# huzaifakhan04/truely-real-time-ai-generated-video-detection-framework-for-social-platforms

Measured on AMD Instinct MI355X. Metric: frames/sec (detect+embed+drift) 720p, higher is better.
Workload: dtype f32; 1 GPU; BASELINE configs[1]: synthetic 720p 1-face frames, batch=256 per GPU, fp32, MTCNN detect + 80x80 crop + InceptionResnetV1 embed + cosine drift score; frames_per_gpu=256, height=720, width=1280, weights=seeded synthetic (no checkpoints offline), prelu_slopes=unit, min_face_size=20, pyramid_levels=11, valid_faces=256, score=6, emb_crc32=3015932725, mode=sharded, ingest=resident, parallelism=single GPU, batches_in_flight=1, driver=single, embed_group=8

## Files before the change

__graft_entry__.py:

```python
import os
import subprocess
import sys

ROOT = os.path.dirname(os.path.abspath(__file__))
PKG = os.path.join(ROOT, "truely-real-time-ai-generated-video-detection-framework-for-social-platforms_amd")
if ROOT not in sys.path:
    sys.path.insert(0, ROOT)


def build() -> None:
    subprocess.check_call(["make", "-C", os.path.join(PKG, "csrc"), "-j4", "-s"])
    subprocess.check_call(["make", "-C", os.path.join(ROOT, "oracle"), "-s"])
    import truely_amd
    from truely_amd import _lib
    lib = _lib.load()
    missing = [n for n in _lib.EXPORTS if not hasattr(lib, n)]
    if missing:
        raise RuntimeError(f"libtruely_hip.so lacks {missing}")


def smoke() -> None:
    import numpy as np
    import torch
    import truely_amd
    from truely_amd.engine import Engine
    from oracle.oracle import Oracle
    assert torch.cuda.is_available(), "smoke() needs cuda:0"
    torch.cuda.set_device(0)
    blob = truely_amd.weights.synthetic_blob(0)
    eng = Engine(blob, device=0)
    frames = truely_amd.synthetic.synthetic_frames(4, 180, 320, seed=3)
    out = eng.detect_embed(frames)
    d = eng.drift_score(out["emb"], out["valid"], 16, 30)
    ref = Oracle(blob).detect_embed(frames)
    assert np.array_equal(out["valid"].cpu().numpy(), ref["valid"]), "valid mask differs from the oracle"
    assert np.array_equal(out["rect"].cpu().numpy(), ref["rect"]), "crop rectangles differ from the oracle"
    err = float(np.abs(out["emb"].cpu().numpy() - ref["emb"]).max())
    assert err <= 1e-4, f"embedding error {err}"
    assert "libtruely_hip.so" in open("/proc/self/maps").read()
    print(f"smoke ok: {int(ref['valid'].sum())}/4 faces, max |emb - oracle| = {err:.3g}, score = {d['score']}")


if __name__ == "__main__":
    build()
# ... 3 lines not shown
```

include/truely_hip.h:

```cpp
#ifndef TRUELY_HIP_H
#define TRUELY_HIP_H
#include <stddef.h>
#include <stdint.h>

#ifdef __cplusplus
extern "C" {
#endif

#define TRL_ABI_VERSION 7

typedef enum {
    TRL_OK = 0,
    TRL_ERR_INVALID = -1,
    TRL_ERR_HIP = -2,
    TRL_ERR_WEIGHTS = -3,
    TRL_ERR_CAPACITY = -4,
    TRL_ERR_STATE = -5
} trl_status;

typedef struct trl_ctx trl_ctx;

typedef struct {
    int    device;
    int    min_face_size;
// ... 41 lines not shown
                      void* stream);

int  trl_detect_crop(trl_ctx* ctx, const uint8_t* d_frames, int n, int H, int W,
                     float* d_box, float* d_prob, int32_t* d_rect, uint8_t* d_valid, float* d_faces, void* stream);
int  trl_facenet_embed_masked(trl_ctx* ctx, const float* d_faces, const uint8_t* d_valid, int n, int h, int w, float* d_emb, void* stream);

int  trl_detect_embed_begin(trl_ctx* ctx, const uint8_t* d_frames, int n, int H, int W,
                            float* d_box, float* d_prob, int32_t* d_rect, uint8_t* d_valid, float* d_emb, void* stream);
int  trl_detect_crop_begin(trl_ctx* ctx, const uint8_t* d_frames, int n, int H, int W,
                           float* d_box, float* d_prob, int32_t* d_rect, uint8_t* d_valid, float* d_faces, void* stream);
int  trl_detect_embed_end(trl_ctx* ctx);

int  trl_drift_score(trl_ctx* ctx, const float* d_emb, const uint8_t* d_valid, int n,
                     long long frame_count, int fps, float* d_sims, uint8_t* d_flags,
                     int32_t* d_result, void* stream);

#define TRL_DRIFT_STATE_BYTES 2064
int  trl_drift_update(trl_ctx* ctx, void* d_state, const float* d_emb, const uint8_t* d_valid, int n,
                      long long frame_count, int fps, float* d_sims, uint8_t* d_flags, int32_t* d_result, void* stream);

int  trl_ingest_nv12(trl_ctx* ctx, const uint8_t* d_nv12, int n_in, int H, int W, int step,
                     uint8_t* d_bgr, int* n_out, void* stream);
int  trl_ingest_i420(trl_ctx* ctx, const uint8_t* d_i420, int n_in, int H, int W, int step,
                     uint8_t* d_bgr, int* n_out, void* stream);

int  trl_debug_stage_boxes(trl_ctx* ctx, int stage, int frame, float* h_boxes, int max_rows, int* n_out);
int  trl_debug_level_counts(trl_ctx* ctx, int frame, int32_t* h_cand, int32_t* h_keep, int* n_levels);
int  trl_debug_level_cands(trl_ctx* ctx, int frame, int level, void* h_rows, int max_rows, int* n_out);
int  trl_debug_level_keep(trl_ctx* ctx, int frame, int level, int32_t* h_idx, int max_rows, int* n_out);
int  trl_debug_nms_tiers(trl_ctx* ctx, int small_tier, int full_tier);
int  trl_debug_list_stats(trl_ctx* ctx, long long* h_out8);
int  trl_debug_option(trl_ctx* ctx, const char* key, int value);
int  trl_debug_pnet_screen_bound(trl_ctx* ctx, float* A, float* B, int* on);
int  trl_debug_batch_capacity(trl_ctx* ctx, float t2_per_frame, float t3_per_frame, int* last_attempts);
int  trl_debug_pyramid_level(trl_ctx* ctx, const uint8_t* d_frame, int H, int W, int level, float* d_out, int* h, int* w, void* stream);
int  trl_debug_pyramid_batch(trl_ctx* ctx, const uint8_t* d_frames, int n, int H, int W, float* d_out, long long* pyr_stride,
                             int32_t* h_levels, int max_levels, int* n_levels, void* stream);
#define TRL_PYR_PLAN_COLS 6
enum { TRL_PYR_FINE = 1, TRL_PYR_S4 = 2, TRL_PYR_S8 = 3, TRL_PYR_SW4 = 4, TRL_PYR_SW8 = 5,
       TRL_PYR_L0_3 = 6, TRL_PYR_L0_4 = 7, TRL_PYR_L0_5 = 8, TRL_PYR_L1 = 9, TRL_PYR_L2 = 10 };
int  trl_debug_pyramid_plan(trl_ctx* ctx, int32_t* h_rows, int max_levels, int* n_levels);
enum { TRL_FNK_FN_CONV = 1, TRL_FNK_FN_SPLIT4 = 2, TRL_FNK_CONV_TAP = 3, TRL_FNK_IGEMM_VEC = 4, TRL_FNK_IGEMM_SCALAR = 5,
       TRL_FNK_SPLITK4 = 6, TRL_FNK_SPLITK4_TAP = 7, TRL_FNK_TAP48 = 8, TRL_FNK_BF16 = 9 };
typedef struct {
    int32_t conv, family, bm, bn, bk, pad, nz, m, cout, k, precision, has_res;
    char layer[48];
} trl_fn_plan_row;
int  trl_debug_facenet_plan(trl_ctx* ctx, trl_fn_plan_row* h_rows, int max_rows, int* n_rows);
int  trl_debug_facenet_capture(trl_ctx* ctx, int conv_index);
int  trl_debug_facenet_capture_read(trl_ctx* ctx, int view, void* h_dst, size_t max_bytes, int32_t* dims5);
int  trl_debug_poison(trl_ctx* ctx, int byte);
int  trl_debug_pnet_level(trl_ctx* ctx, const uint8_t* d_frame, int H, int W, int level,
                          float* d_prob, float* d_reg, int* oh, int* ow, void* stream);
int  trl_debug_rnet(trl_ctx* ctx, const float* d_crops, int n, float* d_out, void* stream);
int  trl_debug_onet(trl_ctx* ctx, const float* d_crops, int n, float* d_out, void* stream);
int  trl_debug_front_net(trl_ctx* ctx, const uint8_t* d_frame, int H, int W, const float* h_boxes, int nb, int net,
                         float* d_out, void* stream);
int  trl_debug_stage_net(trl_ctx* ctx, const uint8_t* d_frames, int nf, int H, int W, const float* h_recs, int nb, int net,
                         int capacity, float* d_out, void* stream);
int  trl_debug_front(trl_ctx* ctx, const uint8_t* d_frames, int nf, int H, int W, const int32_t* h_win, int nb, int net,
                     int capacity, float* d_pool, void* stream);
int  trl_debug_lists(trl_ctx* ctx, int kind, int n, int H, int W, const int32_t* h_caps, int n_levels, const int32_t* h_counts,
                     const void* h_rows, const float* h_logits, float* h_pts, float* d_boxes, float* d_probs, float* d_points,
                     int32_t* d_counts, float* d_box0, float* d_prob0, int32_t* d_rect, uint8_t* d_valid, void* stream);
int  trl_debug_mtcnn_plan(trl_ctx* ctx, trl_fn_plan_row* h_rows, int max_rows, int* n_rows);
int  trl_debug_crop_resize(trl_ctx* ctx, const uint8_t* d_frames, int n, int H, int W,
// ... 105 lines not shown
```

truely-real-time-ai-generated-video-detection-framework-for-social-platforms_amd/_lib.py:

```python
from __future__ import annotations

import ctypes as C
import os

_HERE = os.path.dirname(os.path.abspath(__file__))
LIB_PATH = os.path.join(_HERE, "libtruely_hip.so")


class TrlConfig(C.Structure):
    _fields_ = [("device", C.c_int), ("min_face_size", C.c_int), ("thr0", C.c_float), ("thr1", C.c_float),
                ("thr2", C.c_float), ("factor", C.c_double), ("cap_level", C.c_int), ("cap_frame", C.c_int),
                ("max_faces", C.c_int), ("pnet_mode", C.c_int), ("embed_mode", C.c_int), ("embed_precision", C.c_int)]


class TrlJpegdInfo(C.Structure):
    _fields_ = [(n, C.c_int32) for n in ("width", "height", "h_samp", "v_samp", "restart_interval", "scan_offset", "supported", "reason")]


class TrlJpegOptions(C.Structure):
    _fields_ = [(n, C.c_int) for n in ("quality", "subsampling", "restart_rows", "restart_blocks", "optimize")]


class TrlRzHit(C.Structure):
    _fields_ = [("arena", C.c_int32), ("block", C.c_int32), ("site", C.c_char * 24)] + \
# ... 41 lines not shown
    "trl_debug_level_keep": (C.c_int, [_vp, _i, _i, _vp, _i, C.POINTER(_i)]),
    "trl_debug_batch_capacity": (C.c_int, [_vp, _f, _f, C.POINTER(_i)]),
    "trl_debug_nms_tiers": (C.c_int, [_vp, _i, _i]),
    "trl_debug_option": (C.c_int, [_vp, C.c_char_p, _i]),
    "trl_debug_list_stats": (C.c_int, [_vp, C.POINTER(C.c_longlong)]),
    "trl_debug_poison": (C.c_int, [_vp, _i]),
    "trl_debug_pyramid_level": (C.c_int, [_vp, _vp, _i, _i, _i, _vp, C.POINTER(_i), C.POINTER(_i), _vp]),
    "trl_debug_pyramid_batch": (C.c_int, [_vp, _vp, _i, _i, _i, _vp, C.POINTER(C.c_longlong), _vp, _i, C.POINTER(_i), _vp]),
    "trl_debug_pyramid_plan": (C.c_int, [_vp, _vp, _i, C.POINTER(_i)]),
    "trl_debug_facenet_plan": (C.c_int, [_vp, _vp, _i, C.POINTER(_i)]),
    "trl_debug_facenet_capture": (C.c_int, [_vp, _i]),
    "trl_debug_facenet_capture_read": (C.c_int, [_vp, _i, _vp, C.c_size_t, _vp]),
    "trl_debug_pnet_level": (C.c_int, [_vp, _vp, _i, _i, _i, _vp, _vp, C.POINTER(_i), C.POINTER(_i), _vp]),
    "trl_debug_rnet": (C.c_int, [_vp, _vp, _i, _vp, _vp]),
    "trl_debug_onet": (C.c_int, [_vp, _vp, _i, _vp, _vp]),
    "trl_debug_front_net": (C.c_int, [_vp, _vp, _i, _i, _vp, _i, _i, _vp, _vp]),
    "trl_debug_stage_net": (C.c_int, [_vp, _vp, _i, _i, _i, _vp, _i, _i, _i, _vp, _vp]),
    "trl_debug_front": (C.c_int, [_vp, _vp, _i, _i, _i, _vp, _i, _i, _i, _vp, _vp]),
    "trl_debug_mtcnn_plan": (C.c_int, [_vp, _vp, _i, C.POINTER(_i)]),
    "trl_debug_lists": (C.c_int, [_vp, _i, _i, _i, _i, _vp, _i, _vp, _vp, _vp, _vp, _vp, _vp, _vp, _vp, _vp, _vp, _vp, _vp, _vp]),
    "trl_debug_crop_resize": (C.c_int, [_vp, _vp, _i, _i, _i, _vp, _vp, _vp, _vp]),
    "trl_debug_crop_aligned": (C.c_int, [_vp, _vp, _i, _i, _i, _vp, _vp, _i, _i, _vp, _vp]),
    "trl_debug_crop_area": (C.c_int, [_vp, _vp, _i, _i, _i, _vp, _vp, _i, _i, _vp, _vp]),
    "trl_debug_timings": (C.c_int, [_vp, C.POINTER(_f)]),
    "trl_debug_workspace": (C.c_int, [_vp, _i, _i, _i, _i, C.POINTER(C.c_longlong)]),
    "trl_debug_redzone": (C.c_int, [_vp, C.c_longlong, _i]),
    "trl_debug_redzone_report": (C.c_int, [_vp, _i, C.POINTER(C.c_longlong), C.POINTER(TrlRzHit), _i]),
    "trl_debug_redzone_poke": (C.c_int, [_vp, _i, _i, C.c_longlong, _i]),
    "trl_debug_stage_totals": (C.c_int, [_vp, C.POINTER(C.c_int32)]),
    "trl_debug_pnet_run": (C.c_int, [_vp, _i]),
    "trl_debug_pnet_kernel_ms": (C.c_int, [_vp, C.POINTER(C.c_float)]),
    "trl_debug_pnet_span": (C.c_int, [_vp, C.c_int, C.POINTER(C.c_double), C.POINTER(C.c_int32)]),
    "trl_debug_pnet_screen_bound": (C.c_int, [_vp, C.POINTER(_f), C.POINTER(_f), C.POINTER(_i)]),
    "trl_jpeg_create": (C.c_int, [_i, _i, _i, _i, _i, C.POINTER(_vp)]),
    "trl_jpeg_destroy": (C.c_int, [_vp]),
    "trl_jpeg_encode": (C.c_int, [_vp, _vp, _i, C.c_longlong, _vp, C.c_longlong, _vp, _vp]),
    "trl_jpeg_header": (C.c_int, [_i, _i, _i, _vp, C.c_size_t, C.POINTER(_i)]),
    "trl_jpeg_create_ex": (C.c_int, [_i, _i, _i, C.POINTER(TrlJpegOptions), _i, C.POINTER(_vp)]),
    "trl_jpeg_header_ex": (C.c_int, [_i, _i, C.POINTER(TrlJpegOptions), _vp, C.c_size_t, C.POINTER(_i)]),
    "trl_jpeg_optimal_table": (C.c_int, [_vp, _vp, _vp, C.POINTER(_i), C.POINTER(_i)]),
    "trl_jpegd_parse": (C.c_int, [_vp, C.c_size_t, _vp]),
    "trl_jpegd_create": (C.c_int, [_i, _i, _i, _i, C.c_longlong, C.POINTER(_vp)]),
    "trl_jpegd_destroy": (C.c_int, [_vp]),
    "trl_jpegd_debug_poison": (C.c_int, [_vp, _i]),
    "trl_jpegd_decode": (C.c_int, [_vp, _vp, _vp, _vp, _vp, _i, _vp, C.c_longlong, _vp, _vp]),
    "trl_draw_workspace": (C.c_size_t, [_i, _i]),
    "trl_draw": (C.c_int, [_vp, _i, C.c_longlong, _i, _i, _vp, _i, _vp, _i, _vp, C.c_size_t, _vp]),
    "trl_gallery_pack": (C.c_int, [_vp, C.c_longlong, _vp, C.c_longlong, _vp, C.c_longlong, _vp]),
    "trl_gallery_scores": (C.c_int, [_vp, _i, _vp, C.c_longlong, _vp, C.c_longlong, _i, _vp, C.c_longlong, _vp]),
    "trl_gallery_search_workspace": (C.c_size_t, [_i, C.c_longlong, _i, _i]),
    "trl_gallery_search": (C.c_int, [_vp, _vp, _i, _vp, C.c_longlong, _vp, C.c_longlong, _i, _i, _vp, _vp, _vp, C.c_size_t, _i, _vp]),
    "trl_cluster_links": (C.c_int, [_vp, _vp, _i, _vp, C.c_longlong, _vp, _i, _f, _vp, C.c_longlong, _vp, _i, _vp]),
    "trl_cluster_workspace": (C.c_size_t, [_i]),
    "trl_cluster_labels": (C.c_int, [_vp, C.c_longlong, _vp, _i, _i, _vp, _vp, _vp, _vp, C.c_size_t, C.POINTER(_i), _vp]),
    "trl_gallery_hist_workspace": (C.c_size_t, [_i, C.c_longlong, _i, _i]),
    "trl_gallery_hist": (C.c_int, [_vp, _vp, _vp, _i, _vp, C.c_longlong, _vp, _vp, _vp, C.c_longlong, _i, _i, _vp, _i, _vp, _vp, C.c_size_t, _i, _vp]),
    "trl_gallery_range_workspace": (C.c_size_t, [_i, C.c_longlong, _i]),
    "trl_gallery_range_count": (C.c_int, [_vp, _vp, _i, _vp, C.c_longlong, _vp, _vp, C.c_longlong, _i, _f, _i, _vp, _vp, C.c_size_t, _i, _vp]),
    "trl_gallery_range_fill": (C.c_int, [_vp, _vp, _i, _vp, C.c_longlong, _vp, _vp, C.c_longlong, _i, _f, _i, _vp, _vp, C.c_size_t, C.c_longlong,
                                         _vp, _vp, _i, _vp]),
    "trl_gallery_search_groups_workspace": (C.c_size_t, [_i, C.c_longlong, _i, _i]),
    "trl_gallery_search_groups": (C.c_int, [_vp, _vp, _i, _vp, C.c_longlong, _vp, _vp, C.c_longlong, _i, _i, _vp, _vp, _vp, _vp, C.c_size_t,
                                            _i, _vp]),
}
EXPORTS = tuple(_SIGNATURES)


def load(path: str | None = None):
    global _lib
    if _lib is not None:
        return _lib
    path = path or os.environ.get("TRUELY_HIP_LIB") or LIB_PATH
    if not os.path.exists(path):
        raise ImportError(f"{path} not found: build it with `make -C {_HERE}/csrc` "
                          "(or __graft_entry__.build()); there is no CPU fallback")
    try:
        import torch
    except Exception:
        pass
    lib = C.CDLL(path, mode=C.RTLD_GLOBAL)
    for name, (res, args) in _SIGNATURES.items():
        fn = getattr(lib, name)
        fn.restype = res
        fn.argtypes = args
    if lib.trl_abi_version() != 7:
        raise ImportError("libtruely_hip ABI mismatch")
    _lib = lib
    return lib


def check(status: int):
    if status != 0:
        raise TrlError(status, load().trl_last_error().decode(errors="replace"))
```

truely-real-time-ai-generated-video-detection-framework-for-social-platforms_amd/csrc/trl_api.hip:

```cpp
#include <limits.h>
#include <stdarg.h>
#include <stdio.h>
#include <string.h>
#include <stdlib.h>
#include <algorithm>

#include "trl_ctx.h"

static thread_local char g_err[512] = "";
int g_trl_no_fnconv = 0;
int g_trl_pnet_gate = 0;

#include <mutex>
namespace {
std::mutex g_gate_mu;
hipEvent_t g_gate_ev[64] = {};
bool g_gate_set[64] = {};
}
int trl_gate_wait(trl_ctx* c, hipStream_t s) {
    const int d = c->cfg.device;
    if (!g_trl_pnet_gate || d < 0 || d >= 64) return TRL_OK;
    std::lock_guard<std::mutex> lk(g_gate_mu);
    if (g_gate_set[d]) TRL_HIP(hipStreamWaitEvent(s, g_gate_ev[d], 0));
    return TRL_OK;
// ... 890 lines not shown
}
int trl_debug_list_stats(trl_ctx* c, long long* h_out8) {
    if (!c || !h_out8) { trl_set_error("null argument"); return TRL_ERR_INVALID; }
    const int32_t* f = c->h_pinned + 4;
    unsigned long long used = 0;
    memcpy(&used, f + FLG_SPILL_CUR, 8);
    int mx = 0;
    for (int l = 0; l < 32; l++) if (f[FLG_LEVEL_MAX + l] > mx) mx = f[FLG_LEVEL_MAX + l];
    h_out8[0] = c->caps.last_attempts; h_out8[1] = f[FLG_SPILL_LISTS]; h_out8[2] = (long long)used; h_out8[3] = (long long)c->cb.spill_cap;
    h_out8[4] = c->cb.capF; h_out8[5] = c->cb.lay.S; h_out8[6] = mx; h_out8[7] = f[FLG_FRAME_MAX];
    return TRL_OK;
}

int trl_debug_option(trl_ctx* c, const char* key, int value) {
    if (!key) { trl_set_error("null key"); return TRL_ERR_INVALID; }
    if (!strcmp(key, "no_fnconv")) { g_trl_no_fnconv = value ? 1 : 0; return TRL_OK; }
    if (!strcmp(key, "pnet_gate")) { g_trl_pnet_gate = value ? 1 : 0; return TRL_OK; }
    TRL_CHECK(trl_check_idle(c));
    if (!strcmp(key, "rnet_chunk") && value >= 16) { c->rnet_chunk = value; return TRL_OK; }
    if (!strcmp(key, "onet_chunk") && value >= 16) { c->onet_chunk = value; return TRL_OK; }
    if (!strcmp(key, "pnet_screen") && (value == 0 || value == 1)) { c->pnet_screen = value; return TRL_OK; }
    if (!strcmp(key, "pyr_row_bands") && value >= 0) { c->pyr_row_bands = value; return TRL_OK; }
    if (!strcmp(key, "tail_pool") && (value == 0 || value == 1)) { c->tail_pool = value; return TRL_OK; }
    trl_set_error("unknown option '%s' (or value %d out of range)", key, value);
    return TRL_ERR_INVALID;
}

int trl_debug_pnet_screen_bound(trl_ctx* c, float* A, float* B, int* on) {
    if (!c || !A || !B || !on) { trl_set_error("null argument"); return TRL_ERR_INVALID; }
    *A = c->pnet_scrA; *B = c->pnet_scrB; *on = c->pnet_screen_ok && c->pnet_screen;
    return TRL_OK;
}

int trl_debug_batch_capacity(trl_ctx* c, float t2_per_frame, float t3_per_frame, int* last_attempts) {
    if (!c) { trl_set_error("null context"); return TRL_ERR_INVALID; }
    if (t2_per_frame > 0.f) c->caps.t_per_frame[0] = t2_per_frame;
    if (t3_per_frame > 0.f) c->caps.t_per_frame[1] = t3_per_frame;
    if (last_attempts) *last_attempts = c->caps.last_attempts;
    return TRL_OK;
}

int trl_debug_stage_totals(trl_ctx* c, int32_t* h_out2) {
    if (!c || !h_out2) { trl_set_error("null argument"); return TRL_ERR_INVALID; }
    h_out2[0] = c->h_pinned[4 + FLG_T2N]; h_out2[1] = c->h_pinned[4 + FLG_T3N];
    return TRL_OK;
}

int trl_debug_pnet_run(trl_ctx* c, int run) {
    if (!c || run < 0 || run > 64) { trl_set_error("bad argument"); return TRL_ERR_INVALID; }
    c->pnet_run = run;
    return TRL_OK;
}

int trl_debug_pnet_span(trl_ctx* c, int reset, double* ms_sum, int32_t* launches) {
    if (!c || !ms_sum || !launches) { trl_set_error("null argument"); return TRL_ERR_INVALID; }
    *ms_sum = 0.0; *launches = 0;
    if (!c->pnet_clk) return TRL_OK;
    TRL_CHECK(trl_check_idle(c));
    TRL_HIP(hipSetDevice(c->cfg.device));
    TRL_HIP(hipDeviceSynchronize());
    unsigned long long t[2] = {0, 0};
    int khz = 0;
    TRL_HIP(hipMemcpy(t, c->pnet_clk + 36, sizeof t, hipMemcpyDeviceToHost));
    TRL_HIP(hipDeviceGetAttribute(&khz, hipDeviceAttributeWallClockRate, c->cfg.device));
    if (khz > 0) *ms_sum = (double)t[0] / (double)khz;
    *launches = (int32_t)t[1];
// ... 18 lines not shown
```

truely-real-time-ai-generated-video-detection-framework-for-social-platforms_amd/csrc/trl_ctx.h:

```cpp
#pragma once
#include "trl_common.h"
#include "trl_capacity.h"
#include "trl_facenet.h"

struct Cand {
    float x1, y1, x2, y2, score;
    float r0, r1, r2, r3;
    int cell;
};

struct LevelGeom {
    double scale;
    int h, w;
    int oh, ow;
    int chunk;
};

struct CascadeBufs {
    int n = 0, L = 0, H = 0, W = 0;
    LvLayout lay;
    int capF = 0;
    int32_t* lvl_cnt = nullptr;
    Cand* lvl_rec = nullptr;
    int32_t* lvl_keep_cnt = nullptr;
// ... 22 lines not shown
enum { TRL_PNET = 0, TRL_RNET = 1, TRL_ONET = 2 };
extern const NetDesc trl_nets[3];
inline const NetDesc& trl_net_of(int net) { return trl_nets[net == 24 ? TRL_RNET : TRL_ONET]; }
struct NetLayerW { const DevW* w = nullptr; const float* b = nullptr; const float* slope = nullptr; };
struct FnW { const DevW* w = nullptr; const float* scale = nullptr; const float* shift = nullptr; const float* bias = nullptr; };

struct trl_ctx {
    trl_config cfg;
    bool have_weights = false;
    char* wdev = nullptr;
    size_t wbytes = 0;
    std::vector<DevW> wmat;
    NetLayerW mt[3][9];
    FnW fn[FN_ROWS];
    int front_mode[3] = {0, 0, 0};
    const DevW* logits_w = nullptr;
    const float* logits_b = nullptr;
    int num_classes = 0;
    Arena arena;
    Arena scratch;
    size_t arena_need = 0;
    int fn_need_key[6] = {0}; size_t fn_need_bytes = 0;
    Arena sims_tmp;
    int32_t* h_pinned = nullptr;
    CascadeBufs cb;
    LevelGeom lv[32];
    hipEvent_t ev_call0 = nullptr, ev_call1 = nullptr;
    std::vector<std::pair<hipEvent_t, hipEvent_t>> pnet_ev;
    int pnet_ev_used = 0;
    float last_ms[4] = {0, 0, 0, 0};
    int pnet_mono1 = 0;
    int pnet_unit = 0;
    float pnet_scrA = 0.f, pnet_scrB = 0.f;
    int pnet_screen_ok = 0;
    int pnet_screen = 1;
    int pnet_run = 0;
    int32_t* pnet_cursor = nullptr;
    unsigned long long* pnet_clk = nullptr;
    bool pnet_prof = false;
    float pnet_kernel_ms = 0.f;
    int dbg_poison = -1;
    struct RedZone {
        size_t guard = 0; int byte = 0, saved_poison = -1;
        long long sweeps = 0, bytes = 0, nhits = 0;
        std::vector<trl_rz_hit> hits;
        unsigned long long* dev = nullptr; size_t dev_gaps = 0;
    } rz;
    CascadeCaps caps;
    int rnet_chunk = 49152, onet_chunk = 16384;
    int tail_pool = 1;
    int nms_small = 512, nms_full = 2048;
    size_t scratch_after_cascade = 0;
    struct Pending {
        enum Kind { EMBED, CROP, DETECT };
        bool active = false; int attempt = 0; Kind kind = EMBED;
        const uint8_t* frames = nullptr; int n = 0, H = 0, W = 0;
        void* stream = nullptr;
        float* box = nullptr; float* prob = nullptr; int32_t* rect = nullptr; uint8_t* valid = nullptr; float* emb = nullptr;
        float* faces_out = nullptr;
        float* boxes = nullptr; float* probs = nullptr; float* points = nullptr; int32_t* counts = nullptr; int order = 0;
    } pend;
    uint32_t* pyr_tab = nullptr;
    int pyr_tab_H = 0, pyr_tab_W = 0;
    int pyr_row_bands = 0;
    struct { int nlev = 0, own0 = 0, band_cols = 0, strip_rows = 0, n_bands = 0, n_strips = 0; } pyr_fine;
    struct { int L = 0; int32_t row[16][TRL_PYR_PLAN_COLS] = {}; } pyr_plan;
// ... 59 lines not shown
```

truely-real-time-ai-generated-video-detection-framework-for-social-platforms_amd/csrc/trl_pnet.hip:

```cpp
#include "trl_pyramid.h"
#include <stdlib.h>
#include <type_traits>

typedef float f32x4 __attribute__((ext_vector_type(4)));
typedef float f32x16 __attribute__((ext_vector_type(16)));
typedef _Float16 f16x8 __attribute__((ext_vector_type(8)));

namespace {

constexpr int TS = 16;
constexpr int IN_T = 2 * TS + 10;
constexpr int P1_T = TS + 4;
constexpr int C2_T = TS + 2;
constexpr int C2_LD = 17;
constexpr int REGION_A = C2_T * C2_T * C2_LD;
constexpr int REGION_B = P1_T * P1_T * 10 + 224;
static_assert(3 * 7 * 256 <= REGION_A, "input tile (+ the 28 overhang pixels of the 7x256 copy) fits region A");
static_assert(P1_T * P1_T * 10 <= REGION_B, "pooled tile fits region B");
constexpr int SCR_XM = 2 * C2_T * C2_T * 4;
constexpr int CARRY_P = P1_T * 4 * 10;
constexpr int CARRY_C = C2_T * 2 * C2_LD;
constexpr int BAND = 3;
constexpr int VCARRY_P = 4 * P1_T * 10;
constexpr int VCARRY_C = 2 * C2_T * C2_LD;
constexpr int DYN_LDS = (144 * 32 + BAND * (CARRY_P + CARRY_C) + VCARRY_P + VCARRY_C) * 4;
static_assert((144 * 32) % 4 == 0 && CARRY_P % 4 == 0 && CARRY_C % 4 == 0 && VCARRY_P % 4 == 0, "strips stay 16-byte aligned");

struct PLevel {
    int h, w, oh, ow;
    int tiles_x, tile0;
    int tiles_y;
    unsigned bmagic;
    int pix0;
    int kept0[9];
    unsigned txmagic;
    int kept1[19];
    float scale;
    int cap, rec0;
};
static_assert(sizeof(PLevel) == 164 && offsetof(PLevel, txmagic) == 72 && offsetof(PLevel, scale) == 152, "k_pnet_fused's argument layout");
struct PnetArgs {
    const PyrPx* pyr; long long pyr_stride;
    int n_frames, L, tiles_per_frame, H, W;
    unsigned tpf_magic;
    long long kept;
    PLevel lv[16];
    const float *w1, *w2, *w3, *wh;
    const float *b1, *b2, *b3, *bh, *s1, *s2, *s3;
    float thr; int rec_stride;
    float dthr;
    float scrA, scrB; int screen;
    int dbg_skip;
    int32_t* lvl_cnt; Cand* lvl_rec; int32_t* flags;
    int32_t* xcd_next;
    int run;
    unsigned long long* clk;
    int prof;
};


template <int D, int E>
__device__ __forceinline__ int koff(int s, int kq, int e1, int e2, int e3) {
    const int q0 = (4 * s) / D, r0 = (4 * s) % D, thr = D - r0;
    const int add = thr == 1 ? e1 : (thr == 2 ? e2 : (thr == 3 ? e3 : 0));
    return 4 * s + E * q0 + kq + add;
}

template <bool UNIT>
__device__ __forceinline__ float prelu_t(float v, float sl, float sel) { return UNIT ? vmax_nc(v, sl * v) : trl_prelu_med3(v, sl, sel); }
template <bool UNIT>
__device__ __forceinline__ float prelu_pooled_t(float m, float n, float sl, float sel) {
    return UNIT ? vmax_nc(m, sl * (sl < 0.f ? n : m)) : trl_prelu_pooled(m, n, sl, sel);
}

template <int CB, int AB>
__device__ __forceinline__ f32x4 mfma4(float a, float b, f32x4 c) { return __builtin_amdgcn_mfma_f32_4x4x1f32(a, b, c, CB, AB, 0); }
__device__ __forceinline__ void quad_max4(const f32x4& v, float (&o)[4]) {
    float t0, t1, t2, t3;
    asm("v_max_f32_dpp %4, %8, %8 quad_perm:[1,0,3,2] row_mask:0xf bank_mask:0xf\n\t"
        "v_max_f32_dpp %5, %9, %9 quad_perm:[1,0,3,2] row_mask:0xf bank_mask:0xf\n\t"
        "v_max_f32_dpp %6, %10, %10 quad_perm:[1,0,3,2] row_mask:0xf bank_mask:0xf\n\t"
        "v_max_f32_dpp %7, %11, %11 quad_perm:[1,0,3,2] row_mask:0xf bank_mask:0xf\n\t"
        "v_max_f32_dpp %0, %4, %4 quad_perm:[2,3,0,1] row_mask:0xf bank_mask:0xf\n\t"
        "v_max_f32_dpp %1, %5, %5 quad_perm:[2,3,0,1] row_mask:0xf bank_mask:0xf\n\t"
// ... 467 lines not shown
                if (!hasA) {
                } else if (hasB) {
                    accA = __builtin_amdgcn_mfma_f32_16x16x4f32(xa[0], B2[0], bias2v, 0, 0, 0);
                    accB = __builtin_amdgcn_mfma_f32_16x16x4f32(xb[0], B2[0], bias2v, 0, 0, 0);
#pragma unroll
                    for (int s = 1; s < 23; s++) {
                        accA = __builtin_amdgcn_mfma_f32_16x16x4f32(xa[s], B2[s], accA, 0, 0, 0);
                        accB = __builtin_amdgcn_mfma_f32_16x16x4f32(xb[s], B2[s], accB, 0, 0, 0);
                    }
                } else {
                    accA = __builtin_amdgcn_mfma_f32_16x16x4f32(xa[0], B2[0], bias2v, 0, 0, 0);
#pragma unroll
                    for (int s = 1; s < 23; s++) accA = __builtin_amdgcn_mfma_f32_16x16x4f32(xa[s], B2[s], accA, 0, 0, 0);
                }
                __builtin_amdgcn_sched_barrier(0);
                if (j < 2) read_pair2(j + 1);
                __builtin_amdgcn_sched_barrier(0);
#pragma unroll
                for (int q = 0; q < 4; q++) {
                    const int ra = c0 + mtA * 16 + kq * 4 + q;
                    if (hasA && ra < 324) RA[ra * C2_LD + l15] = prelu_t<UNIT>(accA[q], slope2, sel2);
                    const int rb = c0 + mtB * 16 + kq * 4 + q;
                    if (hasB && rb < 324) RA[rb * C2_LD + l15] = prelu_t<UNIT>(accB[q], slope2, sel2);
                }
            }
            }
        }
        if (tid == 0) next_tile_s = t_begin + cursor;
        stamp(4);
        __syncthreads();
        stamp(5);

        if (a.screen) {
            static_assert(SCR_XM + 2 * 324 <= P1_T * P1_T * 10, "fp16 conv2 tile + maxima stay inside the pooled tile");
#pragma unroll
            for (int p = 0; p < 3; p++) {
                int i = ctid + 256 * p;
                if (p == 2) i = i < 2 * 324 ? i : 2 * 324 - 1;
                const float* src = RA + (i < 324 ? i * C2_LD : (i - 324) * C2_LD + 8);
                f16x8 hv;
                float m = 0.f;
#pragma unroll
                for (int j = 0; j < 8; j++) {
                    const float v = src[j];
                    m = fmaxf(m, fabsf(v));
                    hv[j] = (_Float16)v;
                }
                *reinterpret_cast<f16x8*>(RB + 4 * i) = hv;
                RB[SCR_XM + i] = fminf(m, 3.402823466e38f);
                __builtin_amdgcn_sched_barrier(0);
            }
            __syncthreads();
        }

        tile_nxt = __builtin_amdgcn_readfirstlane(next_tile_s);
        if (tile_nxt < t_end) { nxt = decode(tile_nxt); if (!(dbg_skip & 1)) issue_input(nxt); }
        auto strips_get = [&]() __attribute__((always_inline)) {
            if (feeds_next) copy_conv2(std::true_type{}, CC);
            if (feeds_down) copy_rows2(std::true_type{});
        };

        if (!(dbg_skip & 8)) {
            const float fscale = g.scale;
            const f32x4* T3 = reinterpret_cast<const f32x4*>(T3all);
            auto conv3 = [&](int mt, f32x16& P, auto&& between) __attribute__((always_inline)) {
                const int y = mt * 2 + (l31 >> 4), x = l31 & 15;
                const int base = (y * C2_T + x) * C2_LD + hh;
                f32x16 acc;
#pragma unroll
                for (int qa = 0; qa < 4; qa++) {
                    const f32x4 b4 = T3[2 * qa + hh];
                    acc[4 * qa] = b4[0]; acc[4 * qa + 1] = b4[1]; acc[4 * qa + 2] = b4[2]; acc[4 * qa + 3] = b4[3];
                }
                float xa[2][12], wb[2][12];
                auto read_sixth = [&](int sx, float* xo, float* wo) {
#pragma unroll
                    for (int u = 0; u < 12; u++) {
                        const int s = sx * 12 + u, tap = s >> 3, ky = tap / 3, kx = tap - ky * 3;
                        xo[u] = RA[base + (ky * C2_T + kx) * C2_LD + 2 * (s & 7)];
                        wo[u] = B3S[(2 * s + hh) * 32 + l31];
                    }
                };
// ... 44 lines not shown
                        if (p >= a.thr && !(dbg_skip & 32)) {
                            const int seg = f * a.L + l;
                            const int sl = atomicAdd(&a.lvl_cnt[seg], 1);
                            if (sl < a.lv[l].cap) {
                                Cand c;
                                c.x1 = floorf((2.f * (float)ox + 1.f) / fscale);
                                c.y1 = floorf((2.f * (float)oy + 1.f) / fscale);
                                c.x2 = floorf((2.f * (float)ox + 12.f) / fscale);
                                c.y2 = floorf((2.f * (float)oy + 12.f) / fscale);
                                c.score = p;
                                c.r0 = hq[2]; c.r1 = hq[3]; c.r2 = __uint_as_float(u2[1]); c.r3 = __uint_as_float(u3[1]);
                                c.cell = oy * g.ow + ox;
                                a.lvl_rec[(size_t)f * a.rec_stride + a.lv[l].rec0 + sl] = c;
                            } else {
                                a.flags[FLG_LEVEL] = 1;
                            }
                        }
                    }
                }
            };
            const int mt0 = wave, mt1 = wave + 4;
            const bool has0 = 2 * mt0 < vrows, has1 = 2 * mt1 < vrows;
            bool cf0 = has0, cf1 = has1;
            if (has0 && a.screen) {
                const int sb0 = 324 * hh + (mt0 * 2 + (l31 >> 4)) * C2_T + (l31 & 15);
                auto screen = [&](int mt, int sb) __attribute__((always_inline)) {
                    f32x16 S;
#pragma unroll
                    for (int qa = 0; qa < 4; qa++) {
                        const f32x4 b4 = T3[2 * qa + hh];
#pragma unroll
                        for (int qb = 0; qb < 4; qb++) S[4 * qa + qb] = b4[qb];
                    }
                    float xm = 0.f;
#pragma unroll
                    for (int tap = 0; tap < 9; tap++) {
                        const int to = (tap / 3) * C2_T + tap % 3;
                        f16x8 wv;
#pragma unroll
                        for (int j = 0; j < 8; j++) wv[j] = (_Float16)B3S[(tap * 16 + 8 * hh + j) * 32 + l31];
                        const f16x8 xv = *reinterpret_cast<const f16x8*>(RB + 4 * (sb + to));
                        xm = fmaxf(xm, RB[SCR_XM + sb + to]);
                        S = __builtin_amdgcn_mfma_f32_32x32x16_f16(wv, xv, S, 0, 0, 0);
                    }
                    float part = 0.f;
#pragma unroll
                    for (int qa = 0; qa < 4; qa++) {
                        const f32x4 s4 = T3[8 + 2 * qa + hh], w4 = T3[18 + 2 * qa + hh];
#pragma unroll
                        for (int qb = 0; qb < 4; qb++)
                            part = __builtin_fmaf(w4[qb], prelu_t<UNIT>(S[4 * qa + qb], s4[qb], UNIT ? 0.f : trl_prelu_sel(s4[qb])), part);
                    }
                    const auto pp = __builtin_amdgcn_permlane32_swap(__float_as_uint(part), __float_as_uint(part), false, false);
                    const auto px = __builtin_amdgcn_permlane32_swap(__float_as_uint(xm), __float_as_uint(xm), false, false);
                    const float d = (part + __uint_as_float(pp[1])) + T3all[104];
                    const float X = fmaxf(xm, __uint_as_float(px[1]));
                    const float E = __builtin_fmaf(a.scrA, X, a.scrB);
                    const int oy = ty * TS + mt * 2 + (lane >> 4), ox = tx * TS + (lane & 15);
                    const bool hit = !(d + E < a.dthr) || !(fabsf(d) <= 3.402823466e38f) || X > 65504.f;
                    return __builtin_amdgcn_ballot_w64(lane < 32 && oy < g.oh && ox < g.ow && hit) != 0;
                };
                cf0 = screen(mt0, sb0);
                if (has1) cf1 = screen(mt1, sb0 + 8 * C2_T);
                if (DBG) { nscr += has1 ? 2 : 1; ncnf += (cf0 ? 1 : 0) + (cf1 ? 1 : 0); }
            }
            if (cf0 && cf1) {
                f32x16 P0;
                f32x4 hq0 = T3[16 + hh];
                conv3(mt0, P0, [](auto, auto) {});
                {
                    f32x16 P1;
                    f32x4 hq1 = T3[16 + hh];
                    conv3(mt1, P1, [&](auto SX, auto UU) __attribute__((always_inline)) {
                        constexpr int sx = decltype(SX)::value, u = decltype(UU)::value, h = sx * 6 + (u >> 1);
                        if constexpr ((u & 1) == 1 && h < 32) {
                            __builtin_amdgcn_sched_barrier(0);
                            head_step(std::integral_constant<int, h>{}, P0, hq0);
                            __builtin_amdgcn_sched_barrier(0);
                        }
                    });
                    strips_get();
                    heads_all(P1, hq1);
                    emit(mt0, hq0);
                    emit(mt1, hq1);
                }
            } else if (cf0 || cf1) {
                const int mt = cf0 ? mt0 : mt1;
                f32x16 P0;
                f32x4 hq0 = T3[16 + hh];
                conv3(mt, P0, [](auto, auto) {});
                strips_get();
                heads_all(P0, hq0);
                emit(mt, hq0);
            } else {
                strips_get();
            }
        } else {
            strips_get();
        }
        stamp(6);
        __syncthreads();
        stamp(7);
    }
    if (DBG && prof && lane == 0) {
#pragma unroll
        for (int k = 0; k < 8; k++) atomicAdd(&a.clk[2 + 8 * wave + k], pt[k]);
        if (wave == 0) atomicAdd(&a.clk[2 + 32], (unsigned long long)rot);
    }
    if (DBG && lane == 0 && nscr) { atomicAdd(&a.clk[39], (unsigned long long)nscr); atomicAdd(&a.clk[40], (unsigned long long)ncnf); }
    if (DBG && tid == 0) atomicMax(&a.clk[1], (unsigned long long)wall_clock64());
}

}

__global__ void k_pnet_span(unsigned long long* clk) {
    const unsigned long long t0 = clk[0], t1 = clk[1];
    const unsigned long long d = t1 > t0 ? t1 - t0 : 0ull;
    clk[36] += d; clk[37] += 1ull; clk[38] = d;
    clk[0] = ~0ull; clk[1] = 0ull;
}

static void pnet_screen_bound(trl_ctx* c, const float* W, const float* H, const float* b3, const float* s3, const float* bh) {
    c->pnet_screen_ok = 0; c->pnet_scrA = c->pnet_scrB = __builtin_inff();
    for (int i = 0; i < 144 * 32; i++) if (!(fabsf(W[i]) <= 65504.f)) return;
    const double u = ldexp(1.0, -24), uh = ldexp(1.0, -11), tiny = ldexp(1.0, -14);
    auto gamma = [](int n, double uu) { return n * uu / (1.0 - n * uu); };
    const double ge = gamma(145, u), gs = gamma(145, 2 * u), g35 = gamma(35, u), g36 = gamma(36, u);
    double Sa = 0, Sb = fabs((double)bh[0]) + fabs((double)bh[1]);
    double ad = 0, bd = 0, wdP_a = 0, wdP_b = 0;
    for (int co = 0; co < 32; co++) {
        double W1 = 0, D = 0;
        for (int k = 0; k < 144; k++) {
            const double w = W[k * 32 + co], aw = fabs(w);
            W1 += aw;
            D += aw < tiny ? aw : fabs((double)(float)(_Float16)W[k * 32 + co] - w);
        }
        const double b = fabs((double)b3[co]), L = fmax(1.0, fabs((double)s3[co]));
        const double a3 = D * (1 + uh) + W1 * uh + gs * (W1 + D) * (1 + uh) + ge * W1;
        const double b3e = D * tiny + W1 * tiny + gs * (b + (W1 + D) * tiny) + ge * b;
        const double aM = W1 * (1 + ge), bM = b * (1 + ge);
        const double ap = L * (1 + u) * a3 + 2 * u * L * aM, bp = L * (1 + u) * b3e + 2 * u * L * bM;
        const double aP = L * (1 + u) * aM, bP = L * (1 + u) * bM;
        const double w0 = H[co * 32 + 0], w1 = H[co * 32 + 1], wd = fabs(w1 - w0);
        Sa += (fabs(w0) + fabs(w1)) * aP; Sb += (fabs(w0) + fabs(w1)) * bP;
        ad += wd * ap; bd += wd * bp;
        wdP_a += wd * (aP + ap); wdP_b += wd * (bP + bp);
    }
    ad += g36 * (1 + u) * wdP_a;
    bd += g36 * (1 + u) * (fabs((double)bh[1] - (double)bh[0]) + wdP_b);
    const double A = (g35 * Sa + ad) * (1 + ldexp(1.0, -10)), B = (g35 * Sb + bd) * (1 + ldexp(1.0, -10));
    auto up = [](double v) { float f = (float)v; return (double)f < v ? nextafterf(f, __builtin_inff()) : f; };
    c->pnet_scrA = up(A); c->pnet_scrB = up(B); c->pnet_screen_ok = 1;
}

enum { PN_CONV1 = 0, PN_CONV2 = 2, PN_CONV3 = 3, PN_HEADS = 4 };

int trl_pnet_prepare(trl_ctx* c, const char* himg) {
    const NetLayerW* l = c->mt[TRL_PNET];
    auto host = [&](const float* dev) { return trl_host_of(c, himg, dev); };
    c->pnet_mono1 = c->pnet_unit = 1;
    for (int i : {PN_CONV1, PN_CONV2, PN_CONV3}) {
        const float* sl = host(l[i].slope);
        for (int k = 0; k < l[i].w->Cout; k++) {
            if (i == PN_CONV1 && !(sl[k] >= 0.f)) c->pnet_mono1 = 0;
            if (!(sl[k] <= 1.f)) c->pnet_unit = 0;
        }
    }
    pnet_screen_bound(c, host(l[PN_CONV3].w->p), host(l[PN_HEADS].w->p), host(l[PN_CONV3].b), host(l[PN_CONV3].slope), host(l[PN_HEADS].b));
    return TRL_OK;
}

static unsigned sdiv_magic(int d) { return d <= 1 ? 0xFFFFFFFFu : (unsigned)((0x100000000ull + (unsigned)d - 1) / (unsigned)d); }

static void fill_args(trl_ctx* c, int n, int H, int W, const PyrLayout& lay, const PyrPx* pyr, PnetArgs& a) {
    a.pyr = pyr; a.pyr_stride = lay.pyr_stride;
    a.n_frames = n; a.L = lay.L; a.H = H; a.W = W;
    int tiles = 0;
    for (int l = 0; l < lay.L; l++) {
        const LevelGeom& g = c->lv[l];
        PLevel& p = a.lv[l];
        p.h = g.h; p.w = g.w; p.oh = g.oh; p.ow = g.ow;
        p.tiles_x = (g.ow + TS - 1) / TS;
        p.txmagic = sdiv_magic(p.tiles_x);
        p.tile0 = tiles;
        p.tiles_y = (g.oh + TS - 1) / TS;
        p.bmagic = sdiv_magic(BAND * p.tiles_x);
        tiles += p.tiles_x * p.tiles_y;
        p.pix0 = lay.lv[l].pix0;
        p.scale = (float)g.scale;
        p.cap = c->cb.lay.capl[l]; p.rec0 = c->cb.lay.rec0[l];
    }
    a.tiles_per_frame = tiles;
    a.tpf_magic = sdiv_magic(tiles);
    const NetLayerW* l = c->mt[TRL_PNET];
    a.w1 = l[PN_CONV1].w->p; a.w2 = l[PN_CONV2].w->p; a.w3 = l[PN_CONV3].w->p; a.wh = l[PN_HEADS].w->p;
    a.b1 = l[PN_CONV1].b; a.b2 = l[PN_CONV2].b; a.b3 = l[PN_CONV3].b; a.bh = l[PN_HEADS].b;
    a.s1 = l[PN_CONV1].slope; a.s2 = l[PN_CONV2].slope; a.s3 = l[PN_CONV3].slope;
    a.thr = c->cfg.thr0; a.rec_stride = c->cb.lay.S;
    a.dthr = (a.thr >= 0.01f && a.thr <= 0.99f) ? (float)(log((double)a.thr / (1.0 - (double)a.thr)) - 0.05) : -__builtin_inff();
    a.scrA = c->pnet_scrA; a.scrB = c->pnet_scrB; a.screen = c->pnet_screen && c->pnet_screen_ok;
    a.dbg_skip = trl_tune_int("TRL_PNET_SKIP", 0);
    a.lvl_cnt = c->cb.lvl_cnt; a.lvl_rec = c->cb.lvl_rec; a.flags = c->cb.flags;
    a.clk = c->pnet_clk; a.prof = c->pnet_prof ? 1 : 0;
    a.xcd_next = c->pnet_cursor;
}

size_t trl_pnet_fused_bytes(trl_ctx* c, int n, int H, int W) {
    PyrLayout lay;
    if (trl_pyramid_layout(c, H, W, lay) != TRL_OK) return 0;
    return trl_pyramid_bytes(lay, n) + 4096;
}

int trl_pnet_fused_all(trl_ctx* c, const uint8_t* d_frames, int n, int H, int W, hipEvent_t* ev, hipStream_t s) {
    PyrLayout lay;
    PyrPx* pyr = nullptr;
    TRL_CHECK(trl_pyramid_build(c, d_frames, n, H, W, lay, &pyr, ev, s));
    PnetArgs a;
    fill_args(c, n, H, W, lay, pyr, a);
    const int total_tiles = a.tiles_per_frame * n;
    int grid = 256 * 2;
    if (grid > ((total_tiles + 7) / 8) * 8) grid = ((total_tiles + 7) / 8) * 8;
    if (grid < 8) grid = 8;
    TRL_HIP(hipMemsetAsync(c->pnet_cursor, 0, 8 * sizeof(int32_t), s));
    TRL_CHECK(trl_gate_wait(c, s));
    if (ev) TRL_HIP(hipEventRecord(ev[2], s));
#ifdef TRL_TUNING
    const bool dbg = c->pnet_prof || a.dbg_skip || trl_tune_set("TRL_PNET_SPAN");
#else
    const bool dbg = false;
#endif
    const int auto_run = (total_tiles / 8) / 128;
    a.run = c->pnet_run > 0 ? c->pnet_run : (auto_run < 1 ? 1 : (auto_run > 8 * BAND ? 8 * BAND : auto_run));
    auto launch = [&](auto kern) {
// ... 23 lines not shown
```

truely-real-time-ai-generated-video-detection-framework-for-social-platforms_amd/engine.py:

```python
from __future__ import annotations

import ctypes as C
from typing import Optional

import numpy as np
import torch

from . import _lib
from . import weights as _weights


SELECTION_METHODS = {"largest": 0, "probability": 1, "largest_over_threshold": 2, "center_weighted_size": 3}
RESAMPLERS = {"torch": 0, "pil": 1, "cv2": 2}


def _ptr(t: Optional[torch.Tensor]):
    return C.c_void_p(t.data_ptr()) if t is not None else C.c_void_p(0)


class Engine:
    def __init__(self, blob: bytes | None = None, device: int | None = None, pnet_mode: int | None = None,
                 cap_level: int | None = None, cap_frame: int | None = None, min_face_size: int = 20,
                 thresholds=(0.6, 0.7, 0.7), factor: float = 0.709, max_faces: int = 64, embed_mode: int = 0,
                 embed_precision: str | int = 0):
# ... 352 lines not shown
        for v in range(3):
            dims = np.zeros(5, np.int32)
            _lib.check(self.lib.trl_debug_facenet_capture_read(self._h, v, None, 0, dims.ctypes.data_as(C.c_void_p)))
            if dims[3] == 0:
                out.append(None)
                continue
            a = np.empty(tuple(int(d) for d in dims[:4]), np.float32 if dims[4] == 4 else np.uint16)
            _lib.check(self.lib.trl_debug_facenet_capture_read(self._h, v, a.ctypes.data_as(C.c_void_p), a.nbytes,
                                                               dims.ctypes.data_as(C.c_void_p)))
            out.append(a)
        return tuple(out)

    def batch_capacity(self, t2_per_frame: float = 0.0, t3_per_frame: float = 0.0) -> int:
        k = C.c_int()
        _lib.check(self.lib.trl_debug_batch_capacity(self._h, float(t2_per_frame), float(t3_per_frame), C.byref(k)))
        return k.value

    def option(self, key: str, value: int):
        _lib.check(self.lib.trl_debug_option(self._h, key.encode(), int(value)))

    def nms_tiers(self, small: int = 0, full: int = 0):
        _lib.check(self.lib.trl_debug_nms_tiers(self._h, int(small), int(full)))

    def list_stats(self) -> dict:
        t = (C.c_longlong * 8)()
        _lib.check(self.lib.trl_debug_list_stats(self._h, t))
        keys = ("attempts", "spill_lists", "spill_used", "spill_cap", "cap_frame", "slots_per_frame", "max_level_count", "max_frame_total")
        return dict(zip(keys, (int(v) for v in t)))

    def pnet_screen_bound(self):
        A, B, on = C.c_float(), C.c_float(), C.c_int()
        _lib.check(self.lib.trl_debug_pnet_screen_bound(self._h, C.byref(A), C.byref(B), C.byref(on)))
        return float(A.value), float(B.value), bool(on.value)

    def pnet_run(self, run: int = 0):
        _lib.check(self.lib.trl_debug_pnet_run(self._h, int(run)))

    def stage_totals(self):
        t = (C.c_int32 * 2)()
        _lib.check(self.lib.trl_debug_stage_totals(self._h, t))
        return int(t[0]), int(t[1])

    def workspace(self, what: int = 0, n: int = 0, h: int = 0, w: int = 0) -> dict:
        o = (C.c_longlong * 6)()
        _lib.check(self.lib.trl_debug_workspace(self._h, int(what), int(n), int(h), int(w), o))
        return dict(zip(("scratch_cap", "scratch_high", "arena_cap", "arena_off", "arena_need", "need"), (int(v) for v in o)))

    def poison_workspaces(self, byte: int = 0xFF):
        _lib.check(self.lib.trl_debug_poison(self._h, int(byte)))

    def redzone(self, guard: int, byte: int = 0xA5):
        _lib.check(self.lib.trl_debug_redzone(self._h, int(guard), int(byte)))

    def redzone_report(self, clear: bool = False, sweep: bool = False) -> dict:
        o = (C.c_longlong * 4)()
        hits = (_lib.TrlRzHit * 256)()
        _lib.check(self.lib.trl_debug_redzone_report(self._h, (1 if clear else 0) | (2 if sweep else 0), o, hits, 256))
        rows = [dict(arena=int(h.arena), site=h.site.decode(), block=int(h.block), block_bytes=int(h.block_bytes), gap_off=int(h.gap_off),
                     gap_bytes=int(h.gap_bytes), first=int(h.first), last=int(h.last), count=int(h.count)) for h in hits[:int(o[3])]]
        return dict(sweeps=int(o[0]), bytes=int(o[1]), nhits=int(o[2]), hits=rows)

    def redzone_poke(self, arena: int, block: int, offset: int, value: int = 0x3C):
        _lib.check(self.lib.trl_debug_redzone_poke(self._h, int(arena), int(block), int(offset), int(value)))

    def level_counts(self, frame: int):
        a = np.zeros(32, np.int32); b = np.zeros(32, np.int32)
# ... 193 lines not shown
```

Baseline: 22080 frames/s.

## Tighten PNet fp16 screen bound with per-channel weighted error terms

Replaces the PNet fp16 screening error bound, which used a single scalar times the max input magnitude, with a bound built from per-input-channel weights. Each weight is precomputed on the host as the worst case over taps and applied as a weighted sum over tap inputs. A tighter bound should let the screen reject more candidate windows, so fewer of them fall through to the exact fp32 path. The cost is extra FMAs and a larger kernel argument, and correctness depends on the per-channel bound derivation staying rigorous. The build also compiles a second TUNING variant of the library, and the loader tolerates missing debug symbols.

```diff
diff --git a/__graft_entry__.py b/__graft_entry__.py
--- a/__graft_entry__.py
+++ b/__graft_entry__.py
@@ -10,6 +10,7 @@
 
 def build() -> None:
     subprocess.check_call(["make", "-C", os.path.join(PKG, "csrc"), "-j4", "-s"])
+    subprocess.check_call(["make", "-C", os.path.join(PKG, "csrc"), "-j4", "-s", "TUNING=1"])
     subprocess.check_call(["make", "-C", os.path.join(ROOT, "oracle"), "-s"])
     import truely_amd
     from truely_amd import _lib
diff --git a/include/truely_hip.h b/include/truely_hip.h
--- a/include/truely_hip.h
+++ b/include/truely_hip.h
@@ -97,6 +97,7 @@
 int  trl_debug_list_stats(trl_ctx* ctx, long long* h_out8);
 int  trl_debug_option(trl_ctx* ctx, const char* key, int value);
 int  trl_debug_pnet_screen_bound(trl_ctx* ctx, float* A, float* B, int* on);
+int  trl_debug_pnet_screen_weights(trl_ctx* ctx, float* h_g16);
 int  trl_debug_batch_capacity(trl_ctx* ctx, float t2_per_frame, float t3_per_frame, int* last_attempts);
 int  trl_debug_pyramid_level(trl_ctx* ctx, const uint8_t* d_frame, int H, int W, int level, float* d_out, int* h, int* w, void* stream);
 int  trl_debug_pyramid_batch(trl_ctx* ctx, const uint8_t* d_frames, int n, int H, int W, float* d_out, long long* pyr_stride,
diff --git a/truely-real-time-ai-generated-video-detection-framework-for-social-platforms_amd/_lib.py b/truely-real-time-ai-generated-video-detection-framework-for-social-platforms_amd/_lib.py
--- a/truely-real-time-ai-generated-video-detection-framework-for-social-platforms_amd/_lib.py
+++ b/truely-real-time-ai-generated-video-detection-framework-for-social-platforms_amd/_lib.py
@@ -97,6 +97,7 @@
     "trl_debug_pnet_kernel_ms": (C.c_int, [_vp, C.POINTER(C.c_float)]),
     "trl_debug_pnet_span": (C.c_int, [_vp, C.c_int, C.POINTER(C.c_double), C.POINTER(C.c_int32)]),
     "trl_debug_pnet_screen_bound": (C.c_int, [_vp, C.POINTER(_f), C.POINTER(_f), C.POINTER(_i)]),
+    "trl_debug_pnet_screen_weights": (C.c_int, [_vp, C.POINTER(_f)]),
     "trl_jpeg_create": (C.c_int, [_i, _i, _i, _i, _i, C.POINTER(_vp)]),
     "trl_jpeg_destroy": (C.c_int, [_vp]),
     "trl_jpeg_encode": (C.c_int, [_vp, _vp, _i, C.c_longlong, _vp, C.c_longlong, _vp, _vp]),
@@ -145,7 +146,11 @@
         pass
     lib = C.CDLL(path, mode=C.RTLD_GLOBAL)
     for name, (res, args) in _SIGNATURES.items():
-        fn = getattr(lib, name)
+        fn = getattr(lib, name, None)
+        if fn is None and path != LIB_PATH and name.startswith("trl_debug_"):
+            continue
+        if fn is None:
+            raise ImportError(f"{path} lacks {name}")
         fn.restype = res
         fn.argtypes = args
     if lib.trl_abi_version() != 7:
diff --git a/truely-real-time-ai-generated-video-detection-framework-for-social-platforms_amd/csrc/trl_api.hip b/truely-real-time-ai-generated-video-detection-framework-for-social-platforms_amd/csrc/trl_api.hip
--- a/truely-real-time-ai-generated-video-detection-framework-for-social-platforms_amd/csrc/trl_api.hip
+++ b/truely-real-time-ai-generated-video-detection-framework-for-social-platforms_amd/csrc/trl_api.hip
@@ -946,6 +946,12 @@
     return TRL_OK;
 }
 
+int trl_debug_pnet_screen_weights(trl_ctx* c, float* h_g16) {
+    if (!c || !h_g16) { trl_set_error("null argument"); return TRL_ERR_INVALID; }
+    for (int i = 0; i < 16; i++) h_g16[i] = c->pnet_scrG[i];
+    return TRL_OK;
+}
+
 int trl_debug_batch_capacity(trl_ctx* c, float t2_per_frame, float t3_per_frame, int* last_attempts) {
     if (!c) { trl_set_error("null context"); return TRL_ERR_INVALID; }
     if (t2_per_frame > 0.f) c->caps.t_per_frame[0] = t2_per_frame;
diff --git a/truely-real-time-ai-generated-video-detection-framework-for-social-platforms_amd/csrc/trl_ctx.h b/truely-real-time-ai-generated-video-detection-framework-for-social-platforms_amd/csrc/trl_ctx.h
--- a/truely-real-time-ai-generated-video-detection-framework-for-social-platforms_amd/csrc/trl_ctx.h
+++ b/truely-real-time-ai-generated-video-detection-framework-for-social-platforms_amd/csrc/trl_ctx.h
@@ -78,6 +78,7 @@
     int pnet_mono1 = 0;
     int pnet_unit = 0;
     float pnet_scrA = 0.f, pnet_scrB = 0.f;
+    float pnet_scrG[16] = {};
     int pnet_screen_ok = 0;
     int pnet_screen = 1;
     int pnet_run = 0;
diff --git a/truely-real-time-ai-generated-video-detection-framework-for-social-platforms_amd/csrc/trl_pnet.hip b/truely-real-time-ai-generated-video-detection-framework-for-social-platforms_amd/csrc/trl_pnet.hip
--- a/truely-real-time-ai-generated-video-detection-framework-for-social-platforms_amd/csrc/trl_pnet.hip
+++ b/truely-real-time-ai-generated-video-detection-framework-for-social-platforms_amd/csrc/trl_pnet.hip
@@ -49,7 +49,8 @@
     const float *b1, *b2, *b3, *bh, *s1, *s2, *s3;
     float thr; int rec_stride;
     float dthr;
-    float scrA, scrB; int screen;
+    float scrB; int screen;
+    float scrG[16];
     int dbg_skip;
     int32_t* lvl_cnt; Cand* lvl_rec; int32_t* flags;
     int32_t* xcd_next;
@@ -583,22 +584,26 @@
         stamp(5);
 
         if (a.screen) {
-            static_assert(SCR_XM + 2 * 324 <= P1_T * P1_T * 10, "fp16 conv2 tile + maxima stay inside the pooled tile");
+            static_assert(SCR_XM + 2 * 324 <= P1_T * P1_T * 10, "fp16 conv2 tile + error weights stay inside the pooled tile");
 #pragma unroll
             for (int p = 0; p < 3; p++) {
-                int i = ctid + 256 * p;
-                if (p == 2) i = i < 2 * 324 ? i : 2 * 324 - 1;
-                const float* src = RA + (i < 324 ? i * C2_LD : (i - 324) * C2_LD + 8);
+                const int half = p < 2 ? p : wave >> 1;
+                int cell = ctid;
+                if (p == 2) { cell = ctid & 127; cell = 256 + (cell < 324 - 256 ? cell : 324 - 256 - 1); }
+                const int i = 324 * half + cell;
+                const float* src = RA + cell * C2_LD + 8 * half;
+                const float* gs = a.scrG + 8 * half;
                 f16x8 hv;
-                float m = 0.f;
+                float m = 0.f, mx = 0.f;
 #pragma unroll
                 for (int j = 0; j < 8; j++) {
-                    const float v = src[j];
-                    m = fmaxf(m, fabsf(v));
+                    const float v = src[j], av = fabsf(v);
+                    mx = fmaxf(mx, av);
+                    m = __builtin_fmaf(gs[j], av, m);
                     hv[j] = (_Float16)v;
                 }
                 *reinterpret_cast<f16x8*>(RB + 4 * i) = hv;
-                RB[SCR_XM + i] = fminf(m, 3.402823466e38f);
+                RB[SCR_XM + i] = mx > 65504.f ? 3.402823466e38f : fminf(m, 3.402823466e38f);
                 __builtin_amdgcn_sched_barrier(0);
             }
             __syncthreads();
@@ -709,7 +714,7 @@
 #pragma unroll
                         for (int qb = 0; qb < 4; qb++) S[4 * qa + qb] = b4[qb];
                     }
-                    float xm = 0.f;
+                    float em = 0.f;
 #pragma unroll
                     for (int tap = 0; tap < 9; tap++) {
                         const int to = (tap / 3) * C2_T + tap % 3;
@@ -717,7 +722,7 @@
 #pragma unroll
                         for (int j = 0; j < 8; j++) wv[j] = (_Float16)B3S[(tap * 16 + 8 * hh + j) * 32 + l31];
                         const f16x8 xv = *reinterpret_cast<const f16x8*>(RB + 4 * (sb + to));
-                        xm = fmaxf(xm, RB[SCR_XM + sb + to]);
+                        em += RB[SCR_XM + sb + to];
                         S = __builtin_amdgcn_mfma_f32_32x32x16_f16(wv, xv, S, 0, 0, 0);
                     }
                     float part = 0.f;
@@ -729,12 +734,11 @@
                             part = __builtin_fmaf(w4[qb], prelu_t<UNIT>(S[4 * qa + qb], s4[qb], UNIT ? 0.f : trl_prelu_sel(s4[qb])), part);
                     }
                     const auto pp = __builtin_amdgcn_permlane32_swap(__float_as_uint(part), __float_as_uint(part), false, false);
-                    const auto px = __builtin_amdgcn_permlane32_swap(__float_as_uint(xm), __float_as_uint(xm), false, false);
+                    const auto px = __builtin_amdgcn_permlane32_swap(__float_as_uint(em), __float_as_uint(em), false, false);
                     const float d = (part + __uint_as_float(pp[1])) + T3all[104];
-                    const float X = fmaxf(xm, __uint_as_float(px[1]));
-                    const float E = __builtin_fmaf(a.scrA, X, a.scrB);
+                    const float E = (em + __uint_as_float(px[1])) + a.scrB;
                     const int oy = ty * TS + mt * 2 + (lane >> 4), ox = tx * TS + (lane & 15);
-                    const bool hit = !(d + E < a.dthr) || !(fabsf(d) <= 3.402823466e38f) || X > 65504.f;
+                    const bool hit = !(d + E < a.dthr) || !(fabsf(d) <= 3.402823466e38f) || !(E < 3.402823466e38f);
                     return __builtin_amdgcn_ballot_w64(lane < 32 && oy < g.oh && ox < g.ow && hit) != 0;
                 };
                 cf0 = screen(mt0, sb0);
@@ -799,12 +803,14 @@
 
 static void pnet_screen_bound(trl_ctx* c, const float* W, const float* H, const float* b3, const float* s3, const float* bh) {
     c->pnet_screen_ok = 0; c->pnet_scrA = c->pnet_scrB = __builtin_inff();
+    for (int i = 0; i < 16; i++) c->pnet_scrG[i] = __builtin_inff();
     for (int i = 0; i < 144 * 32; i++) if (!(fabsf(W[i]) <= 65504.f)) return;
     const double u = ldexp(1.0, -24), uh = ldexp(1.0, -11), tiny = ldexp(1.0, -14);
     auto gamma = [](int n, double uu) { return n * uu / (1.0 - n * uu); };
     const double ge = gamma(145, u), gs = gamma(145, 2 * u), g35 = gamma(35, u), g36 = gamma(36, u);
     double Sa = 0, Sb = fabs((double)bh[0]) + fabs((double)bh[1]);
     double ad = 0, bd = 0, wdP_a = 0, wdP_b = 0;
+    double g[144] = {};
     for (int co = 0; co < 32; co++) {
         double W1 = 0, D = 0;
         for (int k = 0; k < 144; k++) {
@@ -822,12 +828,23 @@
         Sa += (fabs(w0) + fabs(w1)) * aP; Sb += (fabs(w0) + fabs(w1)) * bP;
         ad += wd * ap; bd += wd * bp;
         wdP_a += wd * (aP + ap); wdP_b += wd * (bP + bp);
+        for (int k = 0; k < 144; k++) {
+            const double w = W[k * 32 + co], aw = fabs(w), Dk = aw < tiny ? aw : fabs((double)(float)(_Float16)W[k * 32 + co] - w);
+            const double a3k = Dk * (1 + uh) + aw * uh + gs * (aw + Dk) * (1 + uh) + ge * aw, aMk = aw * (1 + ge);
+            const double apk = L * (1 + u) * a3k + 2 * u * L * aMk, aPk = L * (1 + u) * aMk;
+            g[k] += g35 * (fabs(w0) + fabs(w1)) * aPk + wd * apk + g36 * (1 + u) * wd * (aPk + apk);
+        }
     }
     ad += g36 * (1 + u) * wdP_a;
     bd += g36 * (1 + u) * (fabs((double)bh[1] - (double)bh[0]) + wdP_b);
     const double A = (g35 * Sa + ad) * (1 + ldexp(1.0, -10)), B = (g35 * Sb + bd) * (1 + ldexp(1.0, -10));
     auto up = [](double v) { float f = (float)v; return (double)f < v ? nextafterf(f, __builtin_inff()) : f; };
     c->pnet_scrA = up(A); c->pnet_scrB = up(B); c->pnet_screen_ok = 1;
+    for (int ci = 0; ci < 16; ci++) {
+        double m = 0;
+        for (int tap = 0; tap < 9; tap++) m = fmax(m, g[tap * 16 + ci]);
+        c->pnet_scrG[ci] = up(m * (1 + ldexp(1.0, -10)));
+    }
 }
 
 enum { PN_CONV1 = 0, PN_CONV2 = 2, PN_CONV3 = 3, PN_HEADS = 4 };
@@ -875,7 +892,8 @@
     a.s1 = l[PN_CONV1].slope; a.s2 = l[PN_CONV2].slope; a.s3 = l[PN_CONV3].slope;
     a.thr = c->cfg.thr0; a.rec_stride = c->cb.lay.S;
     a.dthr = (a.thr >= 0.01f && a.thr <= 0.99f) ? (float)(log((double)a.thr / (1.0 - (double)a.thr)) - 0.05) : -__builtin_inff();
-    a.scrA = c->pnet_scrA; a.scrB = c->pnet_scrB; a.screen = c->pnet_screen && c->pnet_screen_ok;
+    a.scrB = c->pnet_scrB; a.screen = c->pnet_screen && c->pnet_screen_ok;
+    for (int i = 0; i < 16; i++) a.scrG[i] = c->pnet_scrG[i];
     a.dbg_skip = trl_tune_int("TRL_PNET_SKIP", 0);
     a.lvl_cnt = c->cb.lvl_cnt; a.lvl_rec = c->cb.lvl_rec; a.flags = c->cb.flags;
     a.clk = c->pnet_clk; a.prof = c->pnet_prof ? 1 : 0;
diff --git a/truely-real-time-ai-generated-video-detection-framework-for-social-platforms_amd/engine.py b/truely-real-time-ai-generated-video-detection-framework-for-social-platforms_amd/engine.py
--- a/truely-real-time-ai-generated-video-detection-framework-for-social-platforms_amd/engine.py
+++ b/truely-real-time-ai-generated-video-detection-framework-for-social-platforms_amd/engine.py
@@ -408,6 +408,11 @@
         A, B, on = C.c_float(), C.c_float(), C.c_int()
         _lib.check(self.lib.trl_debug_pnet_screen_bound(self._h, C.byref(A), C.byref(B), C.byref(on)))
         return float(A.value), float(B.value), bool(on.value)
+
+    def pnet_screen_weights(self):
+        g = (C.c_float * 16)()
+        _lib.check(self.lib.trl_debug_pnet_screen_weights(self._h, g))
+        return [float(v) for v in g]
 
     def pnet_run(self, run: int = 0):
         _lib.check(self.lib.trl_debug_pnet_run(self._h, int(run)))
```

Measured after the change: 22490 frames/s (median of 6 runs). +1.9%, better.
